# LBANN/DGraph

Hardware: AMD Instinct MI355X
Metric: edges_per_s (higher is better)
Workload: dtype fp32

## Files before the change

### csrc/bindings_f32.cpp

```cpp
#include <algorithm>
#include <mutex>
#include <vector>
#include <set>
#include <tuple>
#include <ATen/ATen.h>
#include <c10/core/DeviceGuard.h>
#include <c10/hip/HIPStream.h>
#include <torch/library.h>

#include "check.h"
#include "kernels/kernels.h"

namespace dgraph {
namespace {

hipStream_t stream_of(const at::Tensor& t) {
  return c10::hip::getCurrentHIPStream(t.device().index()).stream();
}

void same_dev(const at::Tensor& t, const at::Tensor& ref, const char* name) {
  TORCH_CHECK(t.is_cuda() && t.device() == ref.device(), "dgraph_amd: ", name,
              " must be a GPU tensor on ", ref.device());
}

// ... 7 lines not shown
}

const int64_t* idx64(const c10::optional<at::Tensor>& t, const at::Tensor& ref, int64_t n,
                     const char* name) {
  const at::Tensor* p = opt(t);
  if (!p) return nullptr;
  same_dev(*p, ref, name);
  TORCH_CHECK(p->scalar_type() == at::kLong && p->is_contiguous() && p->numel() == n,
              "dgraph_amd: ", name, " must be contiguous int64 with ", n, " entries");
  return p->data_ptr<int64_t>();
}

void spmm_f32_ex_op(const at::Tensor& rowptr, const at::Tensor& col,
                    const c10::optional<at::Tensor>& ew, const c10::optional<at::Tensor>& cs,
                    const c10::optional<at::Tensor>& rs, const c10::optional<at::Tensor>& cmap,
                    const c10::optional<at::Tensor>& row_ids, const at::Tensor& x,
                    const at::Tensor& out, double beta, int64_t cap,
                    const c10::optional<at::Tensor>& row_map,
                    const c10::optional<at::Tensor>& gate,
                    const c10::optional<at::Tensor>& self_add,
                    const c10::optional<at::Tensor>& self_map, int64_t self_row0,
                    const c10::optional<at::Tensor>& rowend,
                    const c10::optional<at::Tensor>& x2, int64_t nsplit, int64_t pass_cols,
                    const c10::optional<at::Tensor>& keep_bits) {
  same_dev(rowptr, x, "rowptr");
  same_dev(col, x, "col");
  same_dev(out, x, "out");
  f32_rows(x, "x");
  f32_rows(out, "out");
  TORCH_CHECK(rowptr.scalar_type() == at::kLong && rowptr.is_contiguous(),
              "rowptr must be contiguous int64");
  TORCH_CHECK(col.is_contiguous() && (col.scalar_type() == at::kInt || col.scalar_type() == at::kLong),
              "col must be contiguous int32/int64");
  TORCH_CHECK(x.size(1) == out.size(1), "x/out feature mismatch");
  const at::Tensor* ri = opt(row_ids);
  const at::Tensor* re = opt(rowend);
  const int64_t csr_rows = re ? re->numel() : rowptr.numel() - 1;
  if (re) {
    same_dev(*re, x, "rowend");
    TORCH_CHECK(re->scalar_type() == at::kLong && re->is_contiguous() &&
                    rowptr.numel() >= re->numel(),
                "rowend must be contiguous int64 with at most rowptr's entries");
  }
  const int64_t nrows = ri ? ri->numel() : csr_rows;
  const int64_t* rid = idx64(row_ids, x, nrows, "row_ids");
  const int64_t* rmap = idx64(row_map, x, nrows, "row_map");
  if (!rmap) TORCH_CHECK(out.size(0) >= nrows, "out has fewer rows than the CSR rows");
// ... 68 lines not shown
      a.self_row0 = self_row0;
    }
  }
  a.row_ids = rid;
  a.row_map = rmap;
  a.x = x.data_ptr<float>();
  a.ldx = x.stride(0);
  a.out = out.data_ptr<float>();
  a.ldo = out.stride(0);
  a.nrows = nrows;
  a.F = static_cast<int>(x.size(1));
  a.beta = static_cast<float>(beta);
  a.cap = cap;
  a.pass_cols = static_cast<int>(pass_cols);
  if (const at::Tensor* kb = opt(keep_bits)) {
    same_dev(*kb, x, "keep_bits");
    TORCH_CHECK(kb->scalar_type() == at::kInt && kb->dim() == 2 && kb->stride(1) == 1,
                "keep_bits must be int32 [rows, words] with unit column stride");
    TORCH_CHECK(kb->size(1) * 32 >= x.size(1), "keep_bits narrower than the columns");
    TORCH_CHECK(kb->size(0) >= (rmap ? out.size(0) : nrows),
                "keep_bits has fewer rows than the output rows");
    a.keep_bits = reinterpret_cast<const uint32_t*>(kb->data_ptr<int32_t>());
    a.ld_bits = kb->stride(0);
  }
  c10::DeviceGuard g(x.device());
  DG_HIP_CHECK(spmm_f32_run(a, stream_of(x)));
}

void gemm_f32_op(const at::Tensor& A1, const at::Tensor& B1, const c10::optional<at::Tensor>& A2,
                 const c10::optional<at::Tensor>& B2, const c10::optional<at::Tensor>& a_rows,
                 const c10::optional<at::Tensor>& bias, const c10::optional<at::Tensor>& cin,
                 double beta, const c10::optional<at::Tensor>& gate,
                 const c10::optional<at::Tensor>& o_rows, bool relu, const at::Tensor& out,
                 const c10::optional<at::Tensor>& row_scale,
                 const c10::optional<at::Tensor>& send_out,
                 const c10::optional<at::Tensor>& send_ptr,
                 const c10::optional<at::Tensor>& send_pos) {
  f32_rows(A1, "A1");
  f32_rows(B1, "B1");
  f32_rows(out, "out");
  same_dev(B1, A1, "B1");
  same_dev(out, A1, "out");
  const at::Tensor* ar = opt(a_rows);
  const int64_t M = ar ? ar->numel() : A1.size(0);
  const int64_t N = B1.size(1), K1 = A1.size(1);
  TORCH_CHECK(B1.size(0) == K1, "gemm_f32: A1/B1 inner dimension mismatch");
// ... 237 lines not shown
void argmax_hits_op(const at::Tensor& z, const at::Tensor& rows, const at::Tensor& y,
                    const at::Tensor& hit, int64_t C) {
  f32_rows(z, "z");
  same_dev(rows, z, "rows");
  same_dev(y, z, "y");
  same_dev(hit, z, "hit");
  const int64_t n = rows.numel();
  TORCH_CHECK(rows.scalar_type() == at::kLong && rows.is_contiguous() &&
                  y.scalar_type() == at::kLong && y.is_contiguous() && y.numel() == n,
              "rows / y must be contiguous int64 of equal length");
  TORCH_CHECK(hit.scalar_type() == at::kByte && hit.is_contiguous() && hit.numel() >= n,
              "hit must be contiguous uint8 with >= n entries");
  TORCH_CHECK(C > 0 && C <= 256 && C <= z.size(1), "argmax_hits: 0 < C <= 256, C <= width");
  c10::DeviceGuard g(z.device());
  DG_HIP_CHECK(argmax_hits(z.data_ptr<float>(), z.stride(0), static_cast<int>(C),
                           rows.data_ptr<int64_t>(), y.data_ptr<int64_t>(), n,
                           hit.data_ptr<uint8_t>(), stream_of(z)));
}

void set_spmm_f32_config_op(int64_t rowgroup, int64_t pass_cols) {
  set_spmm_f32_config(static_cast<int>(rowgroup), static_cast<int>(pass_cols));
}

void set_f32_sched_op(int64_t spmm_grid, int64_t dynamic, int64_t spmm_xcd) {
  if (spmm_grid >= 0) set_spmm_f32_grid(static_cast<int>(spmm_grid));
  if (spmm_xcd >= 0) set_spmm_f32_xcd(static_cast<int>(spmm_xcd));
  if (dynamic >= 0) set_f32_dynamic(dynamic != 0);
}

void f32_init_op() { DG_HIP_CHECK(work_counters_init()); }

}
}

TORCH_LIBRARY_FRAGMENT(dgraph_amd, m) {
  m.def("set_f32_sched(int spmm_grid=-1, int dynamic=-1, int spmm_xcd=-1) -> ()", &dgraph::set_f32_sched_op);
  m.def("f32_init() -> ()", &dgraph::f32_init_op);
  m.def("set_spmm_f32_config(int rowgroup, int pass_cols=-1) -> ()",
        &dgraph::set_spmm_f32_config_op);
  m.def("spmm_f32_ex(Tensor rowptr, Tensor col, Tensor? edge_weight, Tensor? col_scale, "
        "Tensor? row_scale, Tensor? col_map, Tensor? row_ids, Tensor x, Tensor(a!) out, "
        "float beta=0., int cap=0, Tensor? row_map=None, Tensor? gate=None, "
        "Tensor? self_add=None, Tensor? self_map=None, int self_row0=0, Tensor? rowend=None, "
        "Tensor? x2=None, int nsplit=0, int pass_cols=0, Tensor? keep_bits=None) -> ()");
  m.def("gemm_f32(Tensor A1, Tensor B1, Tensor? A2, Tensor? B2, Tensor? a_rows, Tensor? bias, "
        "Tensor? cin, float beta, Tensor? gate, Tensor? o_rows, bool relu, Tensor(a!) out, "
        "Tensor? row_scale=None, Tensor(b!)? send_out=None, Tensor? send_ptr=None, "
        "Tensor? send_pos=None) -> ()");
  m.def("wgrad_f32(Tensor A1, Tensor? A2, Tensor? a1_rows, Tensor G, Tensor(a!) partials, "
        "int blocks, int fresh_from, Tensor(b!)? col_partials=None) -> ()");
  m.def("wgrad_f32_reduce(Tensor partials, Tensor(a!) out) -> ()");
  m.def("row_keep_bits(Tensor h, Tensor? rows, Tensor(a!) bits) -> ()");
  m.def("apply_keep_bits(Tensor(a!) g, Tensor bits, Tensor? rows=None) -> ()");
  m.def("xent_rows(Tensor z, Tensor rows, Tensor y, float scale, Tensor(a!) dz, "
        "Tensor(b!) row_loss, int C) -> ()");
  m.def("argmax_hits(Tensor z, Tensor rows, Tensor y, Tensor(a!) hit, int C) -> ()");
}

TORCH_LIBRARY_IMPL(dgraph_amd, CUDA, m) {
  m.impl("spmm_f32_ex", &dgraph::spmm_f32_ex_op);
  m.impl("gemm_f32", &dgraph::gemm_f32_op);
  m.impl("wgrad_f32", &dgraph::wgrad_f32_op);
  m.impl("wgrad_f32_reduce", &dgraph::wgrad_f32_reduce_op);
  m.impl("row_keep_bits", &dgraph::row_keep_bits_op);
  m.impl("apply_keep_bits", &dgraph::apply_keep_bits_op);
  m.impl("xent_rows", &dgraph::xent_rows_op);
  m.impl("argmax_hits", &dgraph::argmax_hits_op);
// ... 2 lines not shown
```

### csrc/kernels/kernels.h

```cpp
#pragma once
#include <hip/hip_runtime.h>
#include <stdint.h>

#include <initializer_list>

namespace dgraph {

enum class DType : int { F32 = 0, BF16 = 1 };
enum class IType : int { I32 = 0, I64 = 1 };

void set_spmm_config(int variant, int xcd, int pass_cols);

hipError_t spmm_csr(DType dt, IType it, const int64_t* rowptr, const void* col,
                    const float* ew, int heads, int head_dim, const float* col_scale,
                    const float* row_scale, const void* x, int64_t ldx, void* out,
                    int64_t ldo, int64_t nrows, int F, float beta, hipStream_t stream,
                    int64_t cap = 0, const int64_t* row_map = nullptr);

bool spmm_f32_rowgroup_ok(int F, int64_t ldx, int64_t ldo, const void* x, const void* out);
hipError_t spmm_f32_rowgroup(IType it, const int64_t* rowptr, const void* col,
                             const float* ew, const float* col_scale, const float* row_scale,
                             const int32_t* col_map, const int64_t* row_ids, const float* x,
                             int64_t ldx, float* out, int64_t ldo, int64_t nrows, int F,
                             float beta, int64_t cap, const int64_t* row_map,
// ... 13 lines not shown
  const int64_t* row_map = nullptr;
  const float* x = nullptr;
  int64_t ldx = 0;
  const float* x2 = nullptr;
  int64_t ldx2 = 0;
  int64_t nsplit = 0;
  float* out = nullptr;
  int64_t ldo = 0;
  int64_t nrows = 0;
  int F = 0;
  float beta = 0.f;
  int64_t cap = 0;
  const float* gate = nullptr;
  int64_t ldgate = 0;
  const float* self_add = nullptr;
  int64_t ld_self = 0;
  const int32_t* self_map = nullptr;
  int64_t self_row0 = 0;
  int pass_cols = 0;
  int xcd_remap = 0;
  const uint32_t* keep_bits = nullptr;
  int64_t ld_bits = 0;
  int bits_col0 = 0;
};
hipError_t spmm_f32_run(const SpmmF32Args& a, hipStream_t st);
void set_spmm_f32_pass_cols(int cols);
void set_spmm_f32_config(int rowgroup, int pass_cols);
void set_spmm_f32_grid(int blocks);
void set_spmm_f32_xcd(int on);

hipError_t spmm_hub_partials(DType dt, IType it, const int64_t* seg_beg,
                             const int64_t* seg_end, const void* col, const float* ew,
                             const float* col_scale, const void* x, int64_t ldx,
                             float* partials, int64_t nseg, int F, hipStream_t stream);
hipError_t spmm_hub_reduce(DType dt, const float* partials, const int64_t* hub_seg_ptr,
                           const int64_t* hub_rows, const float* row_scale, void* out,
                           int64_t ldo, int64_t nhub, int F, hipStream_t stream);

hipError_t segment_extreme_fwd(DType dt, IType it, bool minimum, const int64_t* rowptr,
                               const void* col, const void* x, int64_t ldx, void* out,
                               int64_t ldo, int32_t* arg, int64_t lda, int64_t nrows, int F,
                               bool second, const int64_t* row_map, hipStream_t stream);
hipError_t segment_extreme_bwd(DType dt, IType it, const int64_t* t_rowptr, const void* t_col,
                               const int32_t* rel, const void* g, int64_t ldg,
                               const int32_t* arg, int64_t lda, void* out, int64_t ldo,
                               int64_t nrows, int F, bool halo, float beta,
                               hipStream_t stream);

hipError_t segment_pna_fwd(IType it, const int64_t* rowptr, const void* col, const float* x,
                           int64_t ldx, float* mean, int64_t ld_mean, float* sdev,
                           int64_t ld_sdev, float* vmax, int64_t ld_vmax, int32_t* amax,
                           int64_t ld_amax, float* vmin, int64_t ld_vmin, int32_t* amin,
// ... 264 lines not shown
```

### csrc/kernels/spmm_f32.hip

```cpp
#include "../common.h"
#include "kernels.h"

namespace dgraph {
namespace {

typedef float f32x2 __attribute__((ext_vector_type(2)));

template <typename IdxT, int LPR, int WMODE, bool CMAP, bool TWO, bool KB = false,
          bool GS = false>
__global__ __launch_bounds__(256) void spmm_f32_rowgroup_kernel(SpmmF32Args a) {
  constexpr int VEC = 4;
  constexpr int G = kWave / LPR;
  constexpr int U = LPR < 8 ? LPR : 8;
  constexpr bool HAS_EW = (WMODE & 1) != 0;
  constexpr bool HAS_CS = (WMODE & 2) != 0;
  const IdxT* __restrict__ col = static_cast<const IdxT*>(a.col);
  const int64_t* __restrict__ rowptr = a.rowptr;
  const int lane = threadIdx.x & (kWave - 1);
  const int g = lane / LPR;
  const int l = lane % LPR;
  const int wv = threadIdx.x >> 6;
  __shared__ uint8_t inv[CMAP ? 4 * 64 : 1];
  const int64_t nrows = a.nrows;
  const int F = a.F;
  const int64_t ngroups = (nrows + G - 1) / G;
  int64_t blk = blockIdx.x;
  if (a.xcd_remap) {
    const int64_t full = static_cast<int64_t>(gridDim.x) & ~int64_t(7);
    if (blk < full) blk = (blk & 7) * (full >> 3) + (blk >> 3);
  }
  const int64_t q0 = (blk * blockDim.x + threadIdx.x) >> 6;
  const int64_t qstep = (static_cast<int64_t>(gridDim.x) * blockDim.x) >> 6;
  const int f = l * VEC;
  const bool active = f < F;
  const float* xf = a.x + (active ? f : 0);
  const float* x2f = TWO ? a.x2 + (active ? f : 0) : nullptr;
  const uint64_t ldx = static_cast<uint64_t>(a.ldx);
  const uint64_t ldx2 = static_cast<uint64_t>(a.ldx2);
  const uint32_t ns = static_cast<uint32_t>(a.nsplit);
  const int cap = a.cap;
  auto row_ptr = [&](uint32_t c) -> const float* {
    if constexpr (TWO) {
      return c < ns ? xf + static_cast<uint64_t>(c) * ldx
                    : x2f + static_cast<uint64_t>(c - ns) * ldx2;
    } else {
      return xf + static_cast<uint64_t>(c) * ldx;
    }
  };
  for (int64_t q = q0; q < ngroups; q += qstep) {
    const int64_t r = q * G + g;
    const bool has_row = r < nrows;
    const int64_t rr = has_row ? (a.row_ids ? a.row_ids[r] : r) : 0;
    const int64_t s = has_row ? rowptr[rr] : 0;
    const int64_t deg1 = has_row ? (a.rowend ? a.rowend[rr] : rowptr[rr + 1]) - s : 0;
    const int deg = static_cast<int>(deg1 > cap ? cap : deg1);
    int32_t m_top = -1;
    if constexpr (GS) m_top = a.self_map[a.self_row0 + (has_row ? r : 0)];
    int maxdeg = deg;
#pragma unroll
    for (int off = LPR; off < kWave; off <<= 1) {
      const int o = __shfl_xor(maxdeg, off, kWave);
      maxdeg = o > maxdeg ? o : maxdeg;
    }
    f32x2 acc[VEC / 2];
#pragma unroll
    for (int i = 0; i < VEC / 2; ++i) acc[i] = f32x2{0.f, 0.f};
    auto load_c = [&](int k) -> int64_t {
      const IdxT c = col[k < deg ? s + k : 0];
      return k < deg ? static_cast<int64_t>(c) : int64_t(0);
    };
    auto load_w = [&](int64_t& c, int k) -> float {
      float w = k < deg ? 1.f : 0.f;
      if constexpr (CMAP) {
        const int32_t m = a.col_map[c];
        w = m >= 0 ? w : 0.f;
        c = m >= 0 ? m : 0;
      }
      if constexpr (HAS_EW) w *= a.ew[k < deg ? s + k : 0];
      if constexpr (HAS_CS) w *= a.col_scale[c];
      return w;
// ... 58 lines not shown
        for (int u = 0; u < U; ++u)
          c[u] = static_cast<uint32_t>(
              __shfl(static_cast<int>(my_c), g * LPR + j0 + u, kWave));
        if (j0 == 0) nx_c = load_c(kn);
#pragma unroll
        for (int u = 0; u < U; ++u) v[u] = *reinterpret_cast<const uint4*>(row_ptr(c[u]));
#pragma unroll
        for (int u = 0; u < U; ++u) w[u] = __shfl(my_w, g * LPR + j0 + u, kWave);
#pragma unroll
        for (int u = 0; u < U; ++u) {
          const f32x2 ww{w[u], w[u]};
          const f32x2 t0{__uint_as_float(v[u].x), __uint_as_float(v[u].y)};
          const f32x2 t1{__uint_as_float(v[u].z), __uint_as_float(v[u].w)};
          acc[0] = __builtin_elementwise_fma(t0, ww, acc[0]);
          acc[1] = __builtin_elementwise_fma(t1, ww, acc[1]);
        }
      }
      my_w = load_w(nx_c, kn);
      my_c = nx_c;
    }
    if (has_row && active) {
      const int64_t orow = (!GS && a.row_map) ? a.row_map[r] : r;
      const float rs = a.row_scale ? a.row_scale[orow] : 1.f;
      float* o = a.out + orow * a.ldo + f;
      const float beta = a.beta;
      float4 res;
      if (beta != 0.f) {
        const float4 old = *reinterpret_cast<const float4*>(o);
        res.x = fmaf(acc[0].x, rs, beta * old.x);
        res.y = fmaf(acc[0].y, rs, beta * old.y);
        res.z = fmaf(acc[1].x, rs, beta * old.z);
        res.w = fmaf(acc[1].y, rs, beta * old.w);
      } else {
        res.x = acc[0].x * rs;
        res.y = acc[0].y * rs;
        res.z = acc[1].x * rs;
        res.w = acc[1].y * rs;
      }
      if constexpr (GS) {
        const float4 sv = *reinterpret_cast<const float4*>(
            a.self_add + static_cast<int64_t>(m_top >= 0 ? m_top : 0) * a.ld_self + f);
        const float4 gv = *reinterpret_cast<const float4*>(a.gate + orow * a.ldgate + f);
        res.x = m_top >= 0 ? res.x + sv.x : res.x;
        res.y = m_top >= 0 ? res.y + sv.y : res.y;
        res.z = m_top >= 0 ? res.z + sv.z : res.z;
        res.w = m_top >= 0 ? res.w + sv.w : res.w;
        res.x = gv.x > 0.f ? res.x : 0.f;
        res.y = gv.y > 0.f ? res.y : 0.f;
        res.z = gv.z > 0.f ? res.z : 0.f;
        res.w = gv.w > 0.f ? res.w : 0.f;
      } else if (a.self_add) {
        const int32_t m = a.self_map[a.self_row0 + orow];
        if (m >= 0) {
          const float4 sv = *reinterpret_cast<const float4*>(a.self_add + m * a.ld_self + f);
          res.x += sv.x;
          res.y += sv.y;
          res.z += sv.z;
          res.w += sv.w;
        }
      }
      if (!GS && a.gate) {
        const float4 gv = *reinterpret_cast<const float4*>(a.gate + orow * a.ldgate + f);
        res.x = gv.x > 0.f ? res.x : 0.f;
        res.y = gv.y > 0.f ? res.y : 0.f;
        res.z = gv.z > 0.f ? res.z : 0.f;
        res.w = gv.w > 0.f ? res.w : 0.f;
      }
      if constexpr (KB) {
        const int c = a.bits_col0 + f;
        const uint32_t w = a.keep_bits[orow * a.ld_bits + (c >> 5)] >> (c & 31);
        res.x = (w & 1u) ? res.x : 0.f;
        res.y = (w & 2u) ? res.y : 0.f;
        res.z = (w & 4u) ? res.z : 0.f;
        res.w = (w & 8u) ? res.w : 0.f;
      }
      *reinterpret_cast<float4*>(o) = res;
    }
  }
}

int g_f32_grid_cap = 0;
int g_f32_xcd = 0;

template <typename IdxT>
hipError_t launch_f32_rg(const SpmmF32Args& a, hipStream_t st) {
  const int lanes = (a.F + 3) / 4;
  const int LPR = lanes <= 8 ? 8 : lanes <= 16 ? 16 : lanes <= 32 ? 32 : 64;
  const int64_t G = kWave / LPR;
  const int64_t ngroups = (a.nrows + G - 1) / G;
  int64_t blocks = (ngroups + 3) / 4;
  SpmmF32Args ka = a;
  ka.xcd_remap = g_f32_xcd ? 1 : 0;
  if (g_f32_grid_cap > 0 && blocks > g_f32_grid_cap) {
    blocks = g_f32_grid_cap;
    ka.xcd_remap = 0;
  }
  if (blocks > 0x7fffffff) return hipErrorInvalidValue;
  const int wmode = (a.ew != nullptr ? 1 : 0) | (a.col_scale != nullptr ? 2 : 0);
  const bool cmap = a.col_map != nullptr;
  const bool two = a.x2 != nullptr;
  const bool kb = a.keep_bits != nullptr;
  if (two && wmode != 0) return hipErrorInvalidValue;
  if (kb && (two || cmap || wmode != 0)) return hipErrorInvalidValue;
  if (kb) {
#define DG_F32_KB(LPR_)                                                                      \
    if (LPR == LPR_) {                                                                       \
      hipLaunchKernelGGL((spmm_f32_rowgroup_kernel<IdxT, LPR_, 0, false, false, true>), grid, \
                         block, 0, st, ka);                                                  \
      return hipGetLastError();                                                              \
    }
    dim3 grid(static_cast<unsigned>(blocks)), block(256);
    DG_F32_KB(8) DG_F32_KB(16) DG_F32_KB(32) DG_F32_KB(64)
#undef DG_F32_KB
    return hipErrorInvalidValue;
  }
  dim3 grid(static_cast<unsigned>(blocks)), block(256);
  if (cmap && wmode == 0 && a.gate && a.self_add && a.self_map && !a.row_map) {
#define DG_F32_GS(LPR_, T_)                                                                    \
    if (LPR == LPR_ && two == T_) {                                                            \
      hipLaunchKernelGGL((spmm_f32_rowgroup_kernel<IdxT, LPR_, 0, true, T_, false, true>), grid, \
                         block, 0, st, ka);                                                    \
      return hipGetLastError();                                                                \
    }
    DG_F32_GS(8, false) DG_F32_GS(16, false) DG_F32_GS(32, false) DG_F32_GS(64, false)
    DG_F32_GS(8, true) DG_F32_GS(16, true) DG_F32_GS(32, true) DG_F32_GS(64, true)
#undef DG_F32_GS
  }
#define DG_F32_K(LPR_, W_, C_, T_)                                                         \
  if (LPR == LPR_ && wmode == W_ && cmap == C_ && two == T_) {                              \
    hipLaunchKernelGGL((spmm_f32_rowgroup_kernel<IdxT, LPR_, W_, C_, T_>), grid, block, 0, \
                       st, ka);                                                             \
    return hipGetLastError();                                                               \
  }
#define DG_F32(LPR_)                                                                        \
  DG_F32_K(LPR_, 0, false, false) DG_F32_K(LPR_, 1, false, false)                           \
  DG_F32_K(LPR_, 2, false, false) DG_F32_K(LPR_, 3, false, false)                           \
  DG_F32_K(LPR_, 0, true, false) DG_F32_K(LPR_, 1, true, false)                             \
  DG_F32_K(LPR_, 2, true, false) DG_F32_K(LPR_, 3, true, false)                             \
  DG_F32_K(LPR_, 0, false, true) DG_F32_K(LPR_, 0, true, true)
  DG_F32(8)
  DG_F32(16)
  DG_F32(32)
  DG_F32(64)
#undef DG_F32_K
#undef DG_F32
  return hipErrorInvalidValue;
}

int g_f32_pass_cols = 64;

}

void set_spmm_f32_pass_cols(int cols) { g_f32_pass_cols = cols > 0 ? cols : 64; }

void set_spmm_f32_grid(int blocks) { g_f32_grid_cap = blocks > 0 ? blocks : 0; }

void set_spmm_f32_xcd(int on) { g_f32_xcd = on ? 1 : 0; }

bool spmm_f32_rowgroup_ok(int F, int64_t ldx, int64_t ldo, const void* x, const void* out) {
  auto al = [](const void* p) { return (reinterpret_cast<uintptr_t>(p) % 16) == 0; };
  return F % 4 == 0 && ldx % 4 == 0 && ldo % 4 == 0 && al(x) && al(out) &&
         ldx < (int64_t(1) << 40);
}

hipError_t spmm_f32_run(const SpmmF32Args& args, hipStream_t st) {
  if (args.nrows <= 0 || args.F <= 0) return hipSuccess;
  auto al = [](const void* p) { return (reinterpret_cast<uintptr_t>(p) & 15) == 0; };
  if (args.self_add && (!args.self_map || !al(args.self_add) || args.ld_self % 4))
    return hipErrorInvalidValue;
  if (args.gate && (!al(args.gate) || args.ldgate % 4)) return hipErrorInvalidValue;
  if (!spmm_f32_rowgroup_ok(args.F, args.ldx, args.ldo, args.x, args.out))
    return hipErrorInvalidValue;
  if (args.x2 && (!al(args.x2) || args.ldx2 % 4 || args.nsplit < 0 ||
                  args.nsplit >= (int64_t(1) << 32)))
    return hipErrorInvalidValue;
  SpmmF32Args a = args;
  a.cap = (args.cap > 0 && args.cap < (int64_t(1) << 30)) ? args.cap : (1 << 30);
  int pc = args.pass_cols > 0 ? args.pass_cols : g_f32_pass_cols;
  pc = pc > 256 ? 256 : (pc < 16 ? 16 : pc - pc % 4);
  for (int c0 = 0; c0 < args.F; c0 += pc) {
    SpmmF32Args p = a;
    p.F = args.F - c0 < pc ? args.F - c0 : pc;
    p.x = args.x + c0;
    p.x2 = args.x2 ? args.x2 + c0 : nullptr;
    p.out = args.out + c0;
    p.gate = args.gate ? args.gate + c0 : nullptr;
    p.self_add = args.self_add ? args.self_add + c0 : nullptr;
    p.bits_col0 = args.bits_col0 + c0;
    const hipError_t err = args.it == IType::I32 ? launch_f32_rg<int32_t>(p, st)
                                                 : launch_f32_rg<int64_t>(p, st);
    if (err != hipSuccess) return err;
  }
  return hipSuccess;
}

hipError_t spmm_f32_rowgroup(IType it, const int64_t* rowptr, const void* col,
                             const float* ew, const float* col_scale, const float* row_scale,
                             const int32_t* col_map, const int64_t* row_ids, const float* x,
                             int64_t ldx, float* out, int64_t ldo, int64_t nrows, int F,
                             float beta, int64_t cap, const int64_t* row_map,
                             hipStream_t st, const float* gate, int64_t ldgate,
                             const float* self_add, int64_t ld_self, const int32_t* self_map,
                             int64_t self_row0) {
  SpmmF32Args a{};
  a.rowptr = rowptr;
  a.col = col;
  a.it = it;
  a.ew = ew;
  a.col_scale = col_scale;
  a.row_scale = row_scale;
  a.col_map = col_map;
  a.row_ids = row_ids;
  a.row_map = row_map;
// ... 19 lines not shown
```

### dgraph_amd/models/sage_fused.py

```python
from __future__ import annotations

import os
from typing import List, Optional, Tuple

import torch

from ..comm.alltoallv import AllToAllV
from ..ops import f32 as F32
from ..ops import kernels as K
from ..parallel.dist_graph import DistGraph
from ..parallel.reorder import graph_locality
from ..utils.config import ExecutorConfig

PLAN_LINK_GBPS = 153.0
PLAN_SPMM_TBPS = 13.0
PLAN_GEMM_TFPS = 120.0
PLAN_HBM_TBPS = 5.0


def _ranges(a: int, b: int, step: int) -> List[Tuple[int, int]]:
    return [(r, min(b, r + step)) for r in range(a, b, step)]


def _pad_to(n: int, m: int) -> int:
# ... 163 lines not shown
            with torch.cuda.device(dev):
                _native.ops().f32_init()
            if os.environ.get("DGRAPH_F32_DYNAMIC") is not None:
                _native.ops().set_f32_sched(-1, int(os.environ["DGRAPH_F32_DYNAMIC"]))
        self.d0_in = x.shape[1]
        self.d0 = _in_width(self.d0_in, len(model.layers))
        if self.d0 != self.d0_in:
            xp = torch.zeros(x.shape[0], self.d0, dtype=x.dtype, device=dev)
            xp[:, :self.d0_in] = x
            x = xp
        self.model, self.g, self.x = model, graph, x.contiguous()
        self.L, self.H = graph.L, graph.H
        self.nl = len(model.layers)
        self.hid = model.layers[0].out_dim
        self.C = model.layers[-1].out_dim
        self.Cp = _width_at_least(self.C, (64, 128, 176, 192, 256))
        self.Cg = _width_at_least(_pad_to(self.C, 32) if self.C > 128 else self.C,
                                  (128, 176, 192, 256))
        self.inv_n = 1.0 / max(int(n_train), 1)
        self._setup_rows(graph, train_idx, y_train, eval_idx, y_eval, eval_is_val)
        self._setup_adjacency(graph, release_graph)
        b = self._plan_memory(graph, reserve_bytes)
        self._plan_chunks(chunk_rows, b)
        self._allocate(graph, b)
        self.row_loss = torch.zeros(self.T.numel(), dtype=torch.float32, device=dev)
        self.hit = torch.zeros(self.E.numel(), dtype=torch.uint8, device=dev)
        self.E_val_l = self.E_val.long()
        self.correct = torch.zeros(2, dtype=torch.long, device=dev)
        self.record = False
        self._events: list = []
        self._packs: dict = {}
        self._agg0_in_h = False
        self._tune_passes()

    def _setup_rows(self, graph: DistGraph, train_idx, y_train, eval_idx, y_eval,
                    eval_is_val) -> None:
        dev, L = self.dev, self.L
        t, tp = torch.sort(train_idx.long())
        self.T, self.yT = t.contiguous(), y_train[tp].contiguous()
        e, ep = torch.sort(eval_idx.long())
        self.E, self.yE = e.contiguous(), y_eval[ep].contiguous()
        self.E_val = eval_is_val[ep].contiguous()
        self.inv_deg = graph.inv_deg
        self.invdegT = self.inv_deg[self.T].contiguous()
        it_t, _, sub = graph._restricted(self.T)
        parts = [self.T, it_t.compact_rows().row_map.long()]
# ... 216 lines not shown
        cr = chunk_rows or self.cfg.chunk_rows
        if cr <= 0:
            cr = int(min(max(spare // per_row, 1 << 16), 1 << 21))
        self.cr = max(256, min(int(cr), max(L, 256)))
        b.note("chunk_arena", self.cr * per_row, True)
        self.memory_plan = b.decisions
        self.chunks = _ranges(0, self.Li, self.cr) + _ranges(self.Li, L, self.cr)
        if not self.chunks:
            self.chunks = [(0, 0)]
        self.nA = sum(1 for r0, r1 in self.chunks if r1 <= self.Li and r1 > r0)
        self.s_chunks = _ranges(0, self.nS, self.cr) or [(0, 0)]
        ss = lambda v, a: int(torch.searchsorted(v, torch.tensor(a, device=v.device)))
        self.ch_T = [(ss(self.T, r0), ss(self.T, r1)) for r0, r1 in self.chunks]
        self.ch_E = [(ss(self.E, r0), ss(self.E, r1)) for r0, r1 in self.chunks]
        self.ch_S = [(ss(self.S, r0), ss(self.S, r1)) for r0, r1 in self.chunks]
        self.ch_Tloc = [(self.T[a:b_] - r0).contiguous()
                        for (r0, _), (a, b_) in zip(self.chunks, self.ch_T)]
        self.ch_Eloc = [(self.E[a:b_] - r0).contiguous()
                        for (r0, _), (a, b_) in zip(self.chunks, self.ch_E)]
        self.ch_Sloc = [(self.S[a:b_] - r0).contiguous()
                        for (r0, _), (a, b_) in zip(self.chunks, self.ch_S)]
        self.ch_send = [self._csr_range(self.send_st, r0, r1) for r0, r1 in self.chunks]

    def _allocate(self, graph: DistGraph, b: "_Budget") -> None:
        cfg, dev, L, H = self.cfg, self.dev, self.L, self.H
        n_send, nT = self.n_send, self.T.numel()
        f = dict(dtype=torch.float32, device=dev)
        self.h = [torch.empty(L, self.hid, **f) for _ in range(self.nl - 1)]
        self.send_buf, self.halo_buf = None, []
        self.ring_send, self.ring_recv = [], []
        self.aS_full = self.gz_full = None
        if graph.send_map is not None and not self.stream:
            self.send_buf = torch.empty(n_send, self.hid, **f)
            self.halo_buf = [torch.empty(H, self.hid, **f) for _ in range(self.nl - 1)]
        elif self.stream:
            blk_s, blk_r = n_send * self.cw, H * self.cw
            ring_fl = max(self.nbuf * (blk_s + blk_r), b.sub_bytes // 4)
            self.ring_arena = torch.empty(ring_fl, **f)
            ra = self.ring_arena
            self.ring_send = [ra[i * blk_s:(i + 1) * blk_s].view(n_send, self.cw)
                              for i in range(self.nbuf)]
            o = self.nbuf * blk_s
            self.ring_recv = [ra[o + i * blk_r:o + (i + 1) * blk_r].view(H, self.cw)
                              for i in range(self.nbuf)]
            self.agg_full = torch.empty(L, max(self.hid, self.d0), **f)
            self.aS_full = torch.empty(self.nS, self.w_lh, **f)
# ... 222 lines not shown
                "boundary_store": dict(self.use_store),
                "halo_stream": ({"column_block": self.cw, "buffers": self.nbuf}
                                if self.stream else False),
                "keep_agg0": self.agg0 is not None, "reuse_agg0": self.reuse_agg0,
                "keep_aS": self.aS_keep is not None,
                "output_self_term_fill": self.zself is not None,
                "compact_T": self.TS is not None,
                "compact_halo_T": self.HTS is not None, "compact_pull": self.PT is not None,
                "support_rows": self.nS,
                "bwd_halo": "pull" if self.pull is not None else "push",
                "output_project_first": self.pf is not None,
                "memory_plan": list(self.memory_plan),
                **({"link_gbps_planned": round(self.link_gbps, 1)}
                   if self.g.send_map is not None else {})}

    def invalidate_input_aggregate(self) -> None:
        self._agg0_in_h = False

    def _gemm(self, A1, B1, A2=None, B2=None, **kw):
        return F32.gemm_f32(A1, B1, A2, B2, **kw)

    def _spmm(self, rowptr, col, x, out=None, **kw):
        kw.setdefault("pass_cols", self.pass_for.get(x.shape[1], 0))
        return F32.spmm_f32(rowptr, col, x, out, **kw)

    def _spmm_u(self, rowptr, col, u, out=None, **kw):
        forced = self.cfg.pass_cols
        w = u.shape[1]
        if forced:
            pc = min(forced, w)
        else:
            base = self.pass_for.get(w, 0)
            frac = self.nS / max(self.L, 1)
            pc = min(w, 256) if (not base or base >= w or frac <= self.cfg.u_full_frac) else base
        kw.setdefault("pass_cols", pc)
        return F32.spmm_f32(rowptr, col, u, out, **kw)

    def _agg(self, hin: torch.Tensor, r0: int, r1: int, out: torch.Tensor, part: str = "all",
             halo: Optional[torch.Tensor] = None, **kw) -> torch.Tensor:
        rp, re = self.adj.rows(r0, r1, part)
        if part != "int" and halo is not None and self.adj.mid is not None:
            kw.update(x2=halo, nsplit=self.L)
        kw.setdefault("row_scale", self.inv_deg[r0:r1])
        return self._spmm(rp, self.adj.col, hin, out, rowend=re, **kw)

    def _tune_passes(self) -> None:
# ... 640 lines not shown
```

### dgraph_amd/ops/f32.py

```python
from __future__ import annotations

import os
from typing import Optional

import torch

from .. import _native



def spmm_f32(rowptr: torch.Tensor, col: torch.Tensor, x: torch.Tensor,
             out: Optional[torch.Tensor] = None, *, row_scale=None, col_scale=None,
             edge_weight=None, col_map: Optional[torch.Tensor] = None,
             row_ids: Optional[torch.Tensor] = None, beta: float = 0.0,
             row_map: Optional[torch.Tensor] = None,
             gate: Optional[torch.Tensor] = None, self_add: Optional[torch.Tensor] = None,
             self_map: Optional[torch.Tensor] = None, self_row0: int = 0,
             pass_cols: int = 0, rowend: Optional[torch.Tensor] = None,
             x2: Optional[torch.Tensor] = None, nsplit: int = 0,
             keep_bits: Optional[torch.Tensor] = None) -> torch.Tensor:
    if row_ids is not None:
        n = row_ids.numel()
    else:
        n = rowend.numel() if rowend is not None else rowptr.numel() - 1
    if out is None:
        if row_map is not None:
            raise ValueError("spmm_f32: row_map needs an explicit out")
        out = torch.empty(n, x.shape[1], dtype=x.dtype, device=x.device)
        beta = 0.0
    if x.is_cuda:
        _native.ops().spmm_f32_ex(rowptr, col, edge_weight, col_scale, row_scale, col_map,
                                  row_ids, x, out, float(beta), 0, row_map, gate, self_add,
                                  self_map, int(self_row0), rowend, x2, int(nsplit),
                                  int(pass_cols), keep_bits)
        return out
    rp = rowptr.long()
    nr = rowend.numel() if rowend is not None else rp.numel() - 1
    rows = torch.arange(nr, device=rp.device) if row_ids is None else row_ids.long()
    beg = rp[rows]
    end = rowend.long()[rows] if rowend is not None else rp[rows + 1]
    deg = end - beg
    seg = torch.repeat_interleave(torch.arange(n, device=rp.device), deg)
    off = torch.zeros(n + 1, dtype=torch.long, device=rp.device)
    torch.cumsum(deg, 0, out=off[1:])
    pos = beg[seg] + (torch.arange(seg.numel(), device=rp.device) - off[:-1][seg])
    c = col.long()[pos]
    w = torch.ones(c.numel(), dtype=torch.float64)
    if edge_weight is not None:
        w = w * edge_weight.double()[pos]
    if col_map is not None:
        c = col_map.long()[c]
        keep = c >= 0
        w = torch.where(keep, w, torch.zeros_like(w))
        c = torch.where(keep, c, torch.zeros_like(c))
    if col_scale is not None:
        w = w * col_scale.double()[c]
    acc = torch.zeros(n, x.shape[1], dtype=torch.float64)
# ... 2 lines not shown
            lo = c < nsplit
            rows_x = torch.empty(c.numel(), x.shape[1], dtype=torch.float64)
            rows_x[lo] = x.double()[c[lo]]
            rows_x[~lo] = x2.double()[c[~lo] - nsplit]
        else:
            rows_x = x.double()[c]
        acc.index_add_(0, seg, rows_x * w.unsqueeze(1))
    o = torch.arange(n) if row_map is None else row_map.long()
    if row_scale is not None:
        acc = acc * row_scale.double()[o].unsqueeze(1)
    if beta != 0.0:
        acc = acc + beta * out[o].double()
    if self_add is not None:
        m = self_map.long()[self_row0 + o]
        add = self_add.double()[m.clamp_min(0)][:, :acc.shape[1]]
        acc = acc + torch.where((m >= 0).unsqueeze(1), add, torch.zeros_like(add))
    if gate is not None:
        acc = torch.where(gate[o][:, :acc.shape[1]] > 0, acc, torch.zeros_like(acc))
    if keep_bits is not None:
        acc = torch.where(unpack_keep_bits(keep_bits[o], acc.shape[1]), acc,
                          torch.zeros_like(acc))
    out[o] = acc.to(out.dtype)
    return out


def unpack_keep_bits(words: torch.Tensor, F: int) -> torch.Tensor:
    sh = torch.arange(32, device=words.device, dtype=torch.int32)
    return (((words.unsqueeze(2) >> sh) & 1) != 0).reshape(words.shape[0], -1)[:, :F]


def gemm_f32_ok(N: int, K1: int, K2: int = 0) -> bool:
    return N in (64, 128, 176, 192, 256) and K1 % 32 == 0 and K1 > 0 and K2 % 32 == 0


def gemm_f32(A1: torch.Tensor, B1: torch.Tensor, A2=None, B2=None, *, a_rows=None, bias=None,
             cin=None, beta: float = 1.0, gate=None, o_rows=None, relu: bool = False,
             out: Optional[torch.Tensor] = None, row_scale=None, send=None) -> torch.Tensor:
    M = a_rows.numel() if a_rows is not None else A1.shape[0]
    N = B1.shape[1]
    if send is not None and o_rows is not None:
        raise ValueError("gemm_f32: send is not combined with o_rows")
    if out is None:
        if o_rows is not None:
            raise ValueError("gemm_f32: o_rows needs an explicit out")
        out = torch.empty(M, N, dtype=torch.float32, device=A1.device)
    if A1.is_cuda:
# ... 352 lines not shown
```

### dgraph_amd/utils/config.py

```python
from __future__ import annotations

import dataclasses
import os
from dataclasses import dataclass, field
from typing import Any, List


@dataclass
class CommConfig:
    backend: str = "nccl"
    overlap: bool = True
    ranks_per_graph: int = -1
    timeout_s: int = 1800
    shmem_transport: str = "auto"


@dataclass
class KernelConfig:
    spmm_variant: int = 4
    spmm_row_map: int = 0
    spmm_pass_cols: int = 128
    spmm_hub_cap: int = 2048
    dual_gemm_variant: int = 2
    halo_chunk_bytes: int = 32 << 20
# ... 30 lines not shown

@dataclass
class ExecutorConfig:
    chunk_rows: int = 0
    overlap: bool = True
    keep_agg0: str = "auto"
    reuse_agg0: str = "auto"
    boundary_store: str = "auto"
    keep_as: str = "auto"
    stream_fill: bool = True
    stream_ramp: bool = False
    stream_out_fill: bool = False
    halo_stream: str = "auto"
    compact_t: str = "off"
    compact_pull: str = "auto"
    pack_stream: str = "compute"
    pack_fused: bool = True
    bwd_halo: str = "pull"
    project_first: str = "auto"
    u_full_frac: float = 0.35
    stream_shapes: str = "64x2,32x2,64x1,32x1"
    pass_cols: int = 0
    plan_link_gbps: float = 0.0

    def __post_init__(self):
        for name, ok in (("keep_agg0", ("auto", "on", "off")),
                         ("reuse_agg0", ("auto", "off")),
                         ("boundary_store", ("auto", "on", "off")),
                         ("keep_as", ("auto", "on", "off")),
                         ("halo_stream", ("auto", "on", "off")),
                         ("compact_t", ("auto", "on", "off")),
                         ("compact_pull", ("auto", "on", "off")),
                         ("pack_stream", ("compute", "comm")),
                         ("bwd_halo", ("pull", "push")),
                         ("project_first", ("auto", "on", "off"))):
            if getattr(self, name) not in ok:
                raise ValueError(f"ExecutorConfig.{name}={getattr(self, name)!r}: one of {ok}")
        self.shapes()

    def shapes(self):
        return tuple(tuple(int(v) for v in t.split("x")) for t in self.stream_shapes.split(","))

    @staticmethod
    def from_env(environ=None) -> "ExecutorConfig":
        env = os.environ if environ is None else environ
        cfg = ExecutorConfig.__new__(ExecutorConfig)
# ... 78 lines not shown
```

Baseline: 5.682 billion.

## Merge SpMM column passes into one launch and schedule long rows first

The f32 SpMM now folds all column passes into a single grid launch, with each block working out its pass and column offset from its block index, instead of issuing one launch per pass. It also precomputes lists of high-degree rows (degree >= 128 by default) per adjacency slice, and gives those rows their own leading blocks so heavy rows start early while regular blocks skip them. The aim is to cut launch overhead and the tail imbalance caused by skewed row degrees. In exchange it adds index arithmetic, extra template variants, and host-side list setup; the merged path drops the grid cap and XCD remap, and weighted SpMM is excluded from both new paths.

Measured after the change: 5.716 billion (median of 6 runs). About the same (+0.6%).

```diff
diff --git a/csrc/bindings_f32.cpp b/csrc/bindings_f32.cpp
--- a/csrc/bindings_f32.cpp
+++ b/csrc/bindings_f32.cpp
@@ -53,7 +53,8 @@
                     const c10::optional<at::Tensor>& self_map, int64_t self_row0,
                     const c10::optional<at::Tensor>& rowend,
                     const c10::optional<at::Tensor>& x2, int64_t nsplit, int64_t pass_cols,
-                    const c10::optional<at::Tensor>& keep_bits) {
+                    const c10::optional<at::Tensor>& keep_bits,
+                    const c10::optional<at::Tensor>& long_rows, int64_t long_thresh) {
   same_dev(rowptr, x, "rowptr");
   same_dev(col, x, "col");
   same_dev(out, x, "out");
@@ -168,6 +169,17 @@
                 "keep_bits has fewer rows than the output rows");
     a.keep_bits = reinterpret_cast<const uint32_t*>(kb->data_ptr<int32_t>());
     a.ld_bits = kb->stride(0);
+  }
+  if (const at::Tensor* lr = opt(long_rows)) {
+    same_dev(*lr, x, "long_rows");
+    TORCH_CHECK(lr->scalar_type() == at::kInt && lr->is_contiguous() && lr->numel() <= nrows,
+                "long_rows must be contiguous int32 with at most one entry per row");
+    TORCH_CHECK(long_thresh > 0, "long_rows needs long_thresh > 0");
+    TORCH_CHECK(!a.ew && !a.col_scale,
+                "long_rows is not combined with edge weights / col_scale");
+    a.long_rows = lr->data_ptr<int32_t>();
+    a.n_long = static_cast<int>(lr->numel());
+    a.long_thresh = long_thresh;
   }
   c10::DeviceGuard g(x.device());
   DG_HIP_CHECK(spmm_f32_run(a, stream_of(x)));
@@ -451,7 +463,9 @@
   set_spmm_f32_config(static_cast<int>(rowgroup), static_cast<int>(pass_cols));
 }
 
-void set_f32_sched_op(int64_t spmm_grid, int64_t dynamic, int64_t spmm_xcd) {
+void set_f32_sched_op(int64_t spmm_grid, int64_t dynamic, int64_t spmm_xcd,
+                      int64_t spmm_merge) {
+  if (spmm_merge >= 0) set_spmm_f32_merge(static_cast<int>(spmm_merge));
   if (spmm_grid >= 0) set_spmm_f32_grid(static_cast<int>(spmm_grid));
   if (spmm_xcd >= 0) set_spmm_f32_xcd(static_cast<int>(spmm_xcd));
   if (dynamic >= 0) set_f32_dynamic(dynamic != 0);
@@ -463,7 +477,8 @@
 }
 
 TORCH_LIBRARY_FRAGMENT(dgraph_amd, m) {
-  m.def("set_f32_sched(int spmm_grid=-1, int dynamic=-1, int spmm_xcd=-1) -> ()", &dgraph::set_f32_sched_op);
+  m.def("set_f32_sched(int spmm_grid=-1, int dynamic=-1, int spmm_xcd=-1, "
+        "int spmm_merge=-1) -> ()", &dgraph::set_f32_sched_op);
   m.def("f32_init() -> ()", &dgraph::f32_init_op);
   m.def("set_spmm_f32_config(int rowgroup, int pass_cols=-1) -> ()",
         &dgraph::set_spmm_f32_config_op);
@@ -471,7 +486,8 @@
         "Tensor? row_scale, Tensor? col_map, Tensor? row_ids, Tensor x, Tensor(a!) out, "
         "float beta=0., int cap=0, Tensor? row_map=None, Tensor? gate=None, "
         "Tensor? self_add=None, Tensor? self_map=None, int self_row0=0, Tensor? rowend=None, "
-        "Tensor? x2=None, int nsplit=0, int pass_cols=0, Tensor? keep_bits=None) -> ()");
+        "Tensor? x2=None, int nsplit=0, int pass_cols=0, Tensor? keep_bits=None, "
+        "Tensor? long_rows=None, int long_thresh=0) -> ()");
   m.def("gemm_f32(Tensor A1, Tensor B1, Tensor? A2, Tensor? B2, Tensor? a_rows, Tensor? bias, "
         "Tensor? cin, float beta, Tensor? gate, Tensor? o_rows, bool relu, Tensor(a!) out, "
         "Tensor? row_scale=None, Tensor(b!)? send_out=None, Tensor? send_ptr=None, "
diff --git a/csrc/kernels/kernels.h b/csrc/kernels/kernels.h
--- a/csrc/kernels/kernels.h
+++ b/csrc/kernels/kernels.h
@@ -59,12 +59,20 @@
   const uint32_t* keep_bits = nullptr;
   int64_t ld_bits = 0;
   int bits_col0 = 0;
+  const int32_t* long_rows = nullptr;
+  int n_long = 0;
+  int64_t long_thresh = 0;
+  int64_t lr_thresh = 0;
+  int npass = 1;
+  uint32_t lr_blocks = 0;
+  uint32_t io_blocks = 0;
 };
 hipError_t spmm_f32_run(const SpmmF32Args& a, hipStream_t st);
 void set_spmm_f32_pass_cols(int cols);
 void set_spmm_f32_config(int rowgroup, int pass_cols);
 void set_spmm_f32_grid(int blocks);
 void set_spmm_f32_xcd(int on);
+void set_spmm_f32_merge(int on);
 
 hipError_t spmm_hub_partials(DType dt, IType it, const int64_t* seg_beg,
                              const int64_t* seg_end, const void* col, const float* ew,
diff --git a/csrc/kernels/spmm_f32.hip b/csrc/kernels/spmm_f32.hip
--- a/csrc/kernels/spmm_f32.hip
+++ b/csrc/kernels/spmm_f32.hip
@@ -7,7 +7,7 @@
 typedef float f32x2 __attribute__((ext_vector_type(2)));
 
 template <typename IdxT, int LPR, int WMODE, bool CMAP, bool TWO, bool KB = false,
-          bool GS = false>
+          bool GS = false, bool LR = false>
 __global__ __launch_bounds__(256) void spmm_f32_rowgroup_kernel(SpmmF32Args a) {
   constexpr int VEC = 4;
   constexpr int G = kWave / LPR;
@@ -22,19 +22,35 @@
   const int wv = threadIdx.x >> 6;
   __shared__ uint8_t inv[CMAP ? 4 * 64 : 1];
   const int64_t nrows = a.nrows;
-  const int F = a.F;
-  const int64_t ngroups = (nrows + G - 1) / G;
+  int pass = 0;
+  bool is_long = false;
   int64_t blk = blockIdx.x;
-  if (a.xcd_remap) {
+  if constexpr (LR) {
+    const uint32_t b = blockIdx.x;
+    const uint32_t nl = static_cast<uint32_t>(a.npass) * a.lr_blocks;
+    is_long = b < nl;
+    const uint32_t per = is_long ? a.lr_blocks : a.io_blocks;
+    uint32_t bb = is_long ? b : b - nl;
+    while (bb >= per) {
+      bb -= per;
+      ++pass;
+    }
+    blk = bb;
+  }
+  const int coff = LR ? pass * a.pass_cols : 0;
+  const int F = LR ? (a.F - coff < a.pass_cols ? a.F - coff : a.pass_cols) : a.F;
+  const int64_t ngroups = ((LR && is_long ? static_cast<int64_t>(a.n_long) : nrows) + G - 1) / G;
+  if (!LR && a.xcd_remap) {
     const int64_t full = static_cast<int64_t>(gridDim.x) & ~int64_t(7);
     if (blk < full) blk = (blk & 7) * (full >> 3) + (blk >> 3);
   }
   const int64_t q0 = (blk * blockDim.x + threadIdx.x) >> 6;
-  const int64_t qstep = (static_cast<int64_t>(gridDim.x) * blockDim.x) >> 6;
+  const int64_t qstep = LR ? (int64_t(1) << 40)
+                           : (static_cast<int64_t>(gridDim.x) * blockDim.x) >> 6;
   const int f = l * VEC;
   const bool active = f < F;
-  const float* xf = a.x + (active ? f : 0);
-  const float* x2f = TWO ? a.x2 + (active ? f : 0) : nullptr;
+  const float* xf = a.x + coff + (active ? f : 0);
+  const float* x2f = TWO ? a.x2 + coff + (active ? f : 0) : nullptr;
   const uint64_t ldx = static_cast<uint64_t>(a.ldx);
   const uint64_t ldx2 = static_cast<uint64_t>(a.ldx2);
   const uint32_t ns = static_cast<uint32_t>(a.nsplit);
@@ -48,14 +64,27 @@
     }
   };
   for (int64_t q = q0; q < ngroups; q += qstep) {
-    const int64_t r = q * G + g;
-    const bool has_row = r < nrows;
+    int64_t r = q * G + g;
+    bool has_row = r < nrows;
+    if constexpr (LR) {
+      if (is_long) {
+        has_row = r < a.n_long;
+        r = has_row ? a.long_rows[r] : 0;
+      }
+    }
     const int64_t rr = has_row ? (a.row_ids ? a.row_ids[r] : r) : 0;
     const int64_t s = has_row ? rowptr[rr] : 0;
-    const int64_t deg1 = has_row ? (a.rowend ? a.rowend[rr] : rowptr[rr + 1]) - s : 0;
+    int64_t deg1 = has_row ? (a.rowend ? a.rowend[rr] : rowptr[rr + 1]) - s : 0;
+    const bool in_rows = has_row;
+    if constexpr (LR) {
+      if (!is_long && deg1 >= a.lr_thresh) {
+        has_row = false;
+        deg1 = 0;
+      }
+    }
     const int deg = static_cast<int>(deg1 > cap ? cap : deg1);
     int32_t m_top = -1;
-    if constexpr (GS) m_top = a.self_map[a.self_row0 + (has_row ? r : 0)];
+    if constexpr (GS) m_top = a.self_map[a.self_row0 + (in_rows ? r : 0)];
     int maxdeg = deg;
 #pragma unroll
     for (int off = LPR; off < kWave; off <<= 1) {
@@ -160,7 +189,7 @@
     if (has_row && active) {
       const int64_t orow = (!GS && a.row_map) ? a.row_map[r] : r;
       const float rs = a.row_scale ? a.row_scale[orow] : 1.f;
-      float* o = a.out + orow * a.ldo + f;
+      float* o = a.out + coff + orow * a.ldo + f;
       const float beta = a.beta;
       float4 res;
       if (beta != 0.f) {
@@ -177,8 +206,9 @@
       }
       if constexpr (GS) {
         const float4 sv = *reinterpret_cast<const float4*>(
-            a.self_add + static_cast<int64_t>(m_top >= 0 ? m_top : 0) * a.ld_self + f);
-        const float4 gv = *reinterpret_cast<const float4*>(a.gate + orow * a.ldgate + f);
+            a.self_add + coff + static_cast<int64_t>(m_top >= 0 ? m_top : 0) * a.ld_self + f);
+        const float4 gv =
+            *reinterpret_cast<const float4*>(a.gate + coff + orow * a.ldgate + f);
         res.x = m_top >= 0 ? res.x + sv.x : res.x;
         res.y = m_top >= 0 ? res.y + sv.y : res.y;
         res.z = m_top >= 0 ? res.z + sv.z : res.z;
@@ -190,7 +220,8 @@
       } else if (a.self_add) {
         const int32_t m = a.self_map[a.self_row0 + orow];
         if (m >= 0) {
-          const float4 sv = *reinterpret_cast<const float4*>(a.self_add + m * a.ld_self + f);
+          const float4 sv =
+              *reinterpret_cast<const float4*>(a.self_add + coff + m * a.ld_self + f);
           res.x += sv.x;
           res.y += sv.y;
           res.z += sv.z;
@@ -198,14 +229,15 @@
         }
       }
       if (!GS && a.gate) {
-        const float4 gv = *reinterpret_cast<const float4*>(a.gate + orow * a.ldgate + f);
+        const float4 gv =
+            *reinterpret_cast<const float4*>(a.gate + coff + orow * a.ldgate + f);
         res.x = gv.x > 0.f ? res.x : 0.f;
         res.y = gv.y > 0.f ? res.y : 0.f;
         res.z = gv.z > 0.f ? res.z : 0.f;
         res.w = gv.w > 0.f ? res.w : 0.f;
       }
       if constexpr (KB) {
-        const int c = a.bits_col0 + f;
+        const int c = a.bits_col0 + coff + f;
         const uint32_t w = a.keep_bits[orow * a.ld_bits + (c >> 5)] >> (c & 31);
         res.x = (w & 1u) ? res.x : 0.f;
         res.y = (w & 2u) ? res.y : 0.f;
@@ -220,16 +252,25 @@
 int g_f32_grid_cap = 0;
 int g_f32_xcd = 0;
 
+int g_f32_merge = 1;
+
 template <typename IdxT>
-hipError_t launch_f32_rg(const SpmmF32Args& a, hipStream_t st) {
-  const int lanes = (a.F + 3) / 4;
+hipError_t launch_f32_rg(const SpmmF32Args& a, hipStream_t st, bool lr) {
+  const int lanes = ((lr && a.pass_cols < a.F ? a.pass_cols : a.F) + 3) / 4;
   const int LPR = lanes <= 8 ? 8 : lanes <= 16 ? 16 : lanes <= 32 ? 32 : 64;
   const int64_t G = kWave / LPR;
   const int64_t ngroups = (a.nrows + G - 1) / G;
   int64_t blocks = (ngroups + 3) / 4;
   SpmmF32Args ka = a;
   ka.xcd_remap = g_f32_xcd ? 1 : 0;
-  if (g_f32_grid_cap > 0 && blocks > g_f32_grid_cap) {
+  if (lr) {
+    const int64_t lgroups = (static_cast<int64_t>(a.n_long) + G - 1) / G;
+    ka.lr_blocks = static_cast<uint32_t>((lgroups + 3) / 4);
+    ka.io_blocks = static_cast<uint32_t>(blocks);
+    ka.lr_thresh = a.n_long > 0 ? a.long_thresh : (int64_t(1) << 62);
+    ka.xcd_remap = 0;
+    blocks = (blocks + ka.lr_blocks) * a.npass;
+  } else if (g_f32_grid_cap > 0 && blocks > g_f32_grid_cap) {
     blocks = g_f32_grid_cap;
     ka.xcd_remap = 0;
   }
@@ -240,48 +281,54 @@
   const bool kb = a.keep_bits != nullptr;
   if (two && wmode != 0) return hipErrorInvalidValue;
   if (kb && (two || cmap || wmode != 0)) return hipErrorInvalidValue;
+  if (lr && wmode != 0) return hipErrorInvalidValue;
+  dim3 grid(static_cast<unsigned>(blocks)), block(256);
+#define DG_F32_LAUNCH(...)                                                                  \
+  {                                                                                         \
+    hipLaunchKernelGGL((spmm_f32_rowgroup_kernel<IdxT, __VA_ARGS__>), grid, block, 0, st, ka); \
+    return hipGetLastError();                                                               \
+  }
   if (kb) {
-#define DG_F32_KB(LPR_)                                                                      \
-    if (LPR == LPR_) {                                                                       \
-      hipLaunchKernelGGL((spmm_f32_rowgroup_kernel<IdxT, LPR_, 0, false, false, true>), grid, \
-                         block, 0, st, ka);                                                  \
-      return hipGetLastError();                                                              \
-    }
-    dim3 grid(static_cast<unsigned>(blocks)), block(256);
+#define DG_F32_KB(LPR_)                                                        \
+    if (LPR == LPR_) {                                                         \
+      if (lr) DG_F32_LAUNCH(LPR_, 0, false, false, true, false, true)          \
+      DG_F32_LAUNCH(LPR_, 0, false, false, true)                               \
+    }
     DG_F32_KB(8) DG_F32_KB(16) DG_F32_KB(32) DG_F32_KB(64)
 #undef DG_F32_KB
     return hipErrorInvalidValue;
   }
-  dim3 grid(static_cast<unsigned>(blocks)), block(256);
   if (cmap && wmode == 0 && a.gate && a.self_add && a.self_map && !a.row_map) {
-#define DG_F32_GS(LPR_, T_)                                                                    \
-    if (LPR == LPR_ && two == T_) {                                                            \
-      hipLaunchKernelGGL((spmm_f32_rowgroup_kernel<IdxT, LPR_, 0, true, T_, false, true>), grid, \
-                         block, 0, st, ka);                                                    \
-      return hipGetLastError();                                                                \
+#define DG_F32_GS(LPR_, T_)                                                    \
+    if (LPR == LPR_ && two == T_) {                                            \
+      if (lr) DG_F32_LAUNCH(LPR_, 0, true, T_, false, true, true)              \
+      DG_F32_LAUNCH(LPR_, 0, true, T_, false, true)                            \
     }
     DG_F32_GS(8, false) DG_F32_GS(16, false) DG_F32_GS(32, false) DG_F32_GS(64, false)
     DG_F32_GS(8, true) DG_F32_GS(16, true) DG_F32_GS(32, true) DG_F32_GS(64, true)
 #undef DG_F32_GS
   }
-#define DG_F32_K(LPR_, W_, C_, T_)                                                         \
-  if (LPR == LPR_ && wmode == W_ && cmap == C_ && two == T_) {                              \
-    hipLaunchKernelGGL((spmm_f32_rowgroup_kernel<IdxT, LPR_, W_, C_, T_>), grid, block, 0, \
-                       st, ka);                                                             \
-    return hipGetLastError();                                                               \
-  }
+#define DG_F32_K(LPR_, W_, C_, T_) \
+  if (!lr && LPR == LPR_ && wmode == W_ && cmap == C_ && two == T_) DG_F32_LAUNCH(LPR_, W_, C_, T_)
+#define DG_F32_L(LPR_, C_, T_)                         \
+  if (lr && LPR == LPR_ && cmap == C_ && two == T_)    \
+    DG_F32_LAUNCH(LPR_, 0, C_, T_, false, false, true)
 #define DG_F32(LPR_)                                                                        \
   DG_F32_K(LPR_, 0, false, false) DG_F32_K(LPR_, 1, false, false)                           \
   DG_F32_K(LPR_, 2, false, false) DG_F32_K(LPR_, 3, false, false)                           \
   DG_F32_K(LPR_, 0, true, false) DG_F32_K(LPR_, 1, true, false)                             \
   DG_F32_K(LPR_, 2, true, false) DG_F32_K(LPR_, 3, true, false)                             \
-  DG_F32_K(LPR_, 0, false, true) DG_F32_K(LPR_, 0, true, true)
+  DG_F32_K(LPR_, 0, false, true) DG_F32_K(LPR_, 0, true, true)                              \
+  DG_F32_L(LPR_, false, false) DG_F32_L(LPR_, true, false)                                  \
+  DG_F32_L(LPR_, false, true) DG_F32_L(LPR_, true, true)
   DG_F32(8)
   DG_F32(16)
   DG_F32(32)
   DG_F32(64)
 #undef DG_F32_K
+#undef DG_F32_L
 #undef DG_F32
+#undef DG_F32_LAUNCH
   return hipErrorInvalidValue;
 }
 
@@ -294,6 +341,8 @@
 void set_spmm_f32_grid(int blocks) { g_f32_grid_cap = blocks > 0 ? blocks : 0; }
 
 void set_spmm_f32_xcd(int on) { g_f32_xcd = on ? 1 : 0; }
+
+void set_spmm_f32_merge(int on) { g_f32_merge = on ? 1 : 0; }
 
 bool spmm_f32_rowgroup_ok(int F, int64_t ldx, int64_t ldo, const void* x, const void* out) {
   auto al = [](const void* p) { return (reinterpret_cast<uintptr_t>(p) % 16) == 0; };
@@ -316,17 +365,33 @@
   a.cap = (args.cap > 0 && args.cap < (int64_t(1) << 30)) ? args.cap : (1 << 30);
   int pc = args.pass_cols > 0 ? args.pass_cols : g_f32_pass_cols;
   pc = pc > 256 ? 256 : (pc < 16 ? 16 : pc - pc % 4);
+  const int npass = (args.F + pc - 1) / pc;
+  const bool i32 = args.it == IType::I32;
+  const bool weighted = args.ew != nullptr || args.col_scale != nullptr;
+  a.n_long = (args.long_rows && args.n_long > 0 && args.long_thresh > 0) ? args.n_long : 0;
+  if (a.n_long > 0 && (weighted || args.nrows >= (int64_t(1) << 31)))
+    return hipErrorInvalidValue;
+  const bool plain_grid = g_f32_grid_cap == 0 && g_f32_xcd == 0 && !weighted;
+  const bool merged = plain_grid && g_f32_merge != 0 && npass > 1;
+  if (merged) {
+    a.pass_cols = pc;
+    a.npass = npass;
+    return i32 ? launch_f32_rg<int32_t>(a, st, true) : launch_f32_rg<int64_t>(a, st, true);
+  }
+  const bool lr = plain_grid && a.n_long > 0;
   for (int c0 = 0; c0 < args.F; c0 += pc) {
     SpmmF32Args p = a;
     p.F = args.F - c0 < pc ? args.F - c0 : pc;
+    p.pass_cols = p.F;
+    p.npass = 1;
     p.x = args.x + c0;
     p.x2 = args.x2 ? args.x2 + c0 : nullptr;
     p.out = args.out + c0;
     p.gate = args.gate ? args.gate + c0 : nullptr;
     p.self_add = args.self_add ? args.self_add + c0 : nullptr;
     p.bits_col0 = args.bits_col0 + c0;
-    const hipError_t err = args.it == IType::I32 ? launch_f32_rg<int32_t>(p, st)
-                                                 : launch_f32_rg<int64_t>(p, st);
+    const hipError_t err = i32 ? launch_f32_rg<int32_t>(p, st, lr)
+                               : launch_f32_rg<int64_t>(p, st, lr);
     if (err != hipSuccess) return err;
   }
   return hipSuccess;
diff --git a/dgraph_amd/models/sage_fused.py b/dgraph_amd/models/sage_fused.py
--- a/dgraph_amd/models/sage_fused.py
+++ b/dgraph_amd/models/sage_fused.py
@@ -209,6 +209,7 @@
         self._setup_adjacency(graph, release_graph)
         b = self._plan_memory(graph, reserve_bytes)
         self._plan_chunks(chunk_rows, b)
+        self._long_setup(b)
         self._allocate(graph, b)
         self.row_loss = torch.zeros(self.T.numel(), dtype=torch.float32, device=dev)
         self.hit = torch.zeros(self.E.numel(), dtype=torch.uint8, device=dev)
@@ -471,6 +472,45 @@
                         for (r0, _), (a, b_) in zip(self.chunks, self.ch_S)]
         self.ch_send = [self._csr_range(self.send_st, r0, r1) for r0, r1 in self.chunks]
 
+    @staticmethod
+    def _long_key(rowptr, rowend, row_ids):
+        return (rowptr.data_ptr(), rowptr.numel(),
+                rowend.data_ptr() if rowend is not None else 0,
+                row_ids.data_ptr() if row_ids is not None else 0,
+                row_ids.numel() if row_ids is not None else 0)
+
+    def _long_setup(self, b: "_Budget") -> None:
+        self._long: dict = {}
+        self.long_rows_listed = 0
+        thr = int(self.cfg.long_rows)
+        if thr <= 0 or self.dev.type != "cuda":
+            return
+
+        def add(rp, re=None, rows=None):
+            self._long[self._long_key(rp, re, rows)] = F32.long_row_list(
+                rp, thr, rowend=re, row_ids=rows)
+
+        for r0, r1 in self.chunks:
+            if r1 <= r0:
+                continue
+            for part in ("all",) if self.adj.mid is None else ("all", "int", "halo"):
+                add(*self.adj.rows(r0, r1, part))
+            for t in (self.TS, self.PT):
+                if t is not None:
+                    add(t[0][r0:r1 + 1])
+        for s0, s1 in self.s_chunks:
+            if s1 > s0:
+                add(self.adj.rp, None, self.S[s0:s1])
+        n = sum(v.numel() for v in self._long.values())
+        b.note("long_row_lists", 4 * n, True)
+        self.long_rows_listed = n
+
+    def _long_kw(self, rowptr, kw: dict) -> None:
+        if self._long and "long_rows" not in kw:
+            lst = self._long.get(self._long_key(rowptr, kw.get("rowend"), kw.get("row_ids")))
+            if lst is not None:
+                kw.update(long_rows=lst, long_thresh=int(self.cfg.long_rows))
+
     def _allocate(self, graph: DistGraph, b: "_Budget") -> None:
         cfg, dev, L, H = self.cfg, self.dev, self.L, self.H
         n_send, nT = self.n_send, self.T.numel()
@@ -739,6 +779,7 @@
 
     def _spmm(self, rowptr, col, x, out=None, **kw):
         kw.setdefault("pass_cols", self.pass_for.get(x.shape[1], 0))
+        self._long_kw(rowptr, kw)
         return F32.spmm_f32(rowptr, col, x, out, **kw)
 
     def _spmm_u(self, rowptr, col, u, out=None, **kw):
diff --git a/dgraph_amd/ops/f32.py b/dgraph_amd/ops/f32.py
--- a/dgraph_amd/ops/f32.py
+++ b/dgraph_amd/ops/f32.py
@@ -18,7 +18,8 @@
              self_map: Optional[torch.Tensor] = None, self_row0: int = 0,
              pass_cols: int = 0, rowend: Optional[torch.Tensor] = None,
              x2: Optional[torch.Tensor] = None, nsplit: int = 0,
-             keep_bits: Optional[torch.Tensor] = None) -> torch.Tensor:
+             keep_bits: Optional[torch.Tensor] = None,
+             long_rows: Optional[torch.Tensor] = None, long_thresh: int = 0) -> torch.Tensor:
     if row_ids is not None:
         n = row_ids.numel()
     else:
@@ -32,7 +33,7 @@
         _native.ops().spmm_f32_ex(rowptr, col, edge_weight, col_scale, row_scale, col_map,
                                   row_ids, x, out, float(beta), 0, row_map, gate, self_add,
                                   self_map, int(self_row0), rowend, x2, int(nsplit),
-                                  int(pass_cols), keep_bits)
+                                  int(pass_cols), keep_bits, long_rows, int(long_thresh))
         return out
     rp = rowptr.long()
     nr = rowend.numel() if rowend is not None else rp.numel() - 1
@@ -81,6 +82,17 @@
                           torch.zeros_like(acc))
     out[o] = acc.to(out.dtype)
     return out
+
+
+def long_row_list(rowptr: torch.Tensor, thresh: int, *, rowend: Optional[torch.Tensor] = None,
+                  row_ids: Optional[torch.Tensor] = None) -> torch.Tensor:
+    rp = rowptr.long()
+    nr = rowend.numel() if rowend is not None else rp.numel() - 1
+    end = rowend.long() if rowend is not None else rp[1:nr + 1]
+    deg = end - rp[:nr]
+    if row_ids is not None:
+        deg = deg[row_ids.long()]
+    return torch.nonzero(deg >= int(thresh)).reshape(-1).to(torch.int32).contiguous()
 
 
 def unpack_keep_bits(words: torch.Tensor, F: int) -> torch.Tensor:
diff --git a/dgraph_amd/utils/config.py b/dgraph_amd/utils/config.py
--- a/dgraph_amd/utils/config.py
+++ b/dgraph_amd/utils/config.py
@@ -76,6 +76,7 @@
     stream_shapes: str = "64x2,32x2,64x1,32x1"
     pass_cols: int = 0
     plan_link_gbps: float = 0.0
+    long_rows: int = 128
 
     def __post_init__(self):
         for name, ok in (("keep_agg0", ("auto", "on", "off")),
```
